# Critical-Infrastructure-Systems-Lab/ldsr

Measured on NVIDIA B200. Metric: EM fits/sec (T~400, restarts x CV folds), higher is better.
Workload: dtype f64

## Files before the change

ldsr_b200/csrc/em_split_kernel.cuh:

```cuda
#pragma once
#include "em_kernel.cuh"

namespace ldsr {

constexpr int SPLIT_NCH = 10;

template <int PQ> __host__ __device__ constexpr int split_nstat() { return 11 + 3 * PQ; }

__host__ __device__ constexpr bool split_w_in_smem(int pq) { return pq <= 4; }
__host__ __device__ inline size_t split_smem_bytes(int pq, int nw, int max_units, int max_uunits) {
    size_t b = 0;
    b += (size_t)max_units * 3 * 32 * 8;
    b += (size_t)2 * nw * 4 * 32 * 8;
    const bool pair = nw % 2 == 0 && nw * (11 + 3 * pq) > 2 * nw * SPLIT_NCH;
    const size_t ch = (size_t)2 * nw * SPLIT_NCH * 32 * 8, st = (size_t)(pair ? nw / 2 : nw) * (11 + 3 * pq) * 32 * 8;
    b += ch > st ? ch : st;
    b += ((size_t)max_units * 4 + 15) & ~size_t(15);
    b += 128;
    b += (size_t)8 * 32 * 8;
    if (split_w_in_smem(pq)) b += (size_t)max_uunits * pq * 32 * 8;
    if (theta_bd_in_smem(pq)) b += (size_t)2 * pq * 32 * 8;
    return b;
}

constexpr int UNIT_M = 1 << 30, UNIT_M1 = 1 << 29, UNIT_US = 1 << 28, UNIT_T0 = UNIT_US - 1;

template <class F> __host__ __device__ inline void split_window_units(int t0, int T, int mseg, int uw, F f) {
    const int end = T < t0 + uw ? T : t0 + uw;
    int t = t0;
    while (t < end) {
        if (t + mseg <= T - 1 && t + mseg <= end) {
            f(t, false);
            t += mseg;
        } else {
            f(t, true);
            t += 1;
        }
    }
}

inline int split_units_upper_bound(const double *y, int T, int mseg, int uw) {
    int n = 0;
    for (int t0 = 0; t0 < T; t0 += uw) {
        bool any = false;
        for (int t = t0; t < T && t < t0 + uw; t++) any = any || (y[t] == y[t]);
        const bool inside = t0 + uw <= T - 1;
        if (!any && inside)
            n += 1;
        else
            split_window_units(t0, T, mseg, uw, [&](int, bool) { n++; });
// ... 82 lines not shown
        const bool obs = (bits >> j) & 1u;
        const double m11 = obs ? k.mc.a11 : k.A2, m12 = obs ? k.mc.a12 : k.Q;
        const double m21 = obs ? k.mc.C2 : 0.0, m22 = obs ? th.R : 1.0;
        nj[j] = n;
        dj[j] = d;
        nn[j] = fma(m11, n, m12 * d);
        dd[j] = fma(m21, n, m22 * d);
        n = nn[j];
        d = dd[j];
    }
    double rho[N], rn[N];
#pragma unroll
    for (int j = 0; j < N; j++) {
        rho[j] = fast_rcp(dd[j]);
        rn[j] = fast_rcp(nn[j]);
    }
#pragma unroll
    for (int j = 0; j < N; j++) {
        const bool obs = (bits >> j) & 1u;
        const double K = obs ? th.C * nj[j] * rho[j] : 0.0;
        const double nu = obs ? th.R * nj[j] : nj[j];
        const double vu = nu * rho[j];
        const double J = k.A * nu * rn[j];
        G.K[j] = K;
        G.rS[j] = obs ? dj[j] * rho[j] : 0.0;
        G.alpha[j] = fma(-k.mc.AC, K, k.A);
        G.J[j] = J;
        G.L[j] = vu * fma(-k.A, J, 1.0);
    }
    G.Vnext = nn[N - 1] * rho[N - 1];
    G.dend = d;
}

template <int PQ, int N>
__device__ __forceinline__ void unit_inputs(const Theta<PQ> &th, unsigned bits, const double *__restrict__ yseg,
                                            const double *__restrict__ useg, const double *__restrict__ vseg,
                                            double (&Bu)[N], double (&ymd)[N], double (&yo)[N],
                                            double (&ur)[N * PQ], double (&vr)[N * PQ]) {
    double yr[N];
    load_vec<N * PQ>(useg, ur);
    load_vec<N * PQ>(vseg, vr);
    load_vec<N>(yseg, yr);
#pragma unroll
    for (int j = 0; j < N; j++) {
        double b = 0.0, dv = 0.0;
#pragma unroll
        for (int i = 0; i < PQ; i++) {
            b = fma(th.b(i), ur[j * PQ + i], b);
            dv = fma(th.d(i), vr[j * PQ + i], dv);
        }
        const bool obs = (bits >> j) & 1u;
        yo[j] = obs ? yr[j] : 0.0;
        Bu[j] = b;
        ymd[j] = yo[j] - dv;
    }
}

struct PieceFwd {
    double Vq, P, q;
    double l0, l1, l2;
    double dprod;
    int shift;
    double PJ, PJ2, G0, GG, Lc;
};

template <int PQ, int UW, int N>
__device__ __forceinline__ void forward_unit_basis(const Theta<PQ> &th, const SplitConst<PQ, UW> &k, unsigned bits,
                                                   const double *__restrict__ yseg, const double *__restrict__ useg,
                                                   const double *__restrict__ vseg, PieceFwd &c) {
    double Bu[N], ymd[N], yo[N];
    {
        double ur[N * PQ], vr[N * PQ];
        unit_inputs<PQ, N>(th, bits, yseg, useg, vseg, Bu, ymd, yo, ur, vr);
    }
    UnitGains<N> G;
    unit_gains<PQ, UW, N>(th, k, bits, c.Vq, G);
    double q[N + 1], P[N + 1];
    q[0] = c.q;
    P[0] = c.P;
#pragma unroll
    for (int j = 0; j < N; j++) {
        const double beta = fma(k.A * G.K[j], ymd[j], Bu[j]);
        q[j + 1] = fma(G.alpha[j], q[j], beta);
        P[j + 1] = G.alpha[j] * P[j];
    }
    double g0[N], gP[N];
#pragma unroll
    for (int j = 0; j < N; j++) {
        const double d0 = fma(-th.C, q[j], ymd[j]);
        const double w0 = G.rS[j] * d0;
        c.l0 = fma(w0, d0, c.l0);
        c.l1 = fma(w0, P[j], c.l1);
        c.l2 = fma(G.rS[j] * P[j], P[j], c.l2);
        const double xu0 = fma(G.K[j], d0, q[j]);
        const double xuP = P[j] * fma(-G.K[j], th.C, 1.0);
        g0[j] = fma(-G.J[j], q[j + 1], xu0);
        gP[j] = fma(-G.J[j], P[j + 1], xuP);
    }
    double pj = c.PJ, pj2 = c.PJ2;
#pragma unroll
    for (int j = 0; j < N; j++) {
        c.G0 = fma(pj, g0[j], c.G0);
        c.GG = fma(pj, gP[j], c.GG);
        c.Lc = fma(pj2, G.L[j], c.Lc);
        pj *= G.J[j];
        pj2 *= G.J[j] * G.J[j];
    }
// ... 52 lines not shown
                lo = fma(k.A, lo, Bu[j]);
                hi = fma(k.A, hi, Bu[4 + j]);
            }
            hh = fma(hh, k.A8, fma(lo, A4, hi));
        }
    }
    if (KEEP_W) {
#pragma unroll
        for (int i = 0; i < PQ; i++) {
            hh = fma(th.b(i), W[i], hh);
            wk[i * 32] = W[i];
        }
    }
    const double AW = k.AW();
    const double qn = fma(AW, c.q, hh);
    const double Pn = AW * c.P;
    const double Vn = fma(k.aVW, c.Vq, k.bVW);
    const double Jc = AW * c.Vq * fast_rcp(Vn);
    const double g0 = fma(-Jc, qn, c.q);
    const double gP = fma(-Jc, Pn, c.P);
    const double L = c.Vq * fma(-AW, Jc, 1.0);
    c.G0 = fma(c.PJ, g0, c.G0);
    c.GG = fma(c.PJ, gP, c.GG);
    c.Lc = fma(c.PJ2, L, c.Lc);
    c.PJ *= Jc;
    c.PJ2 *= Jc * Jc;
    c.q = qn;
    c.P = Pn;
    c.Vq = Vn;
}

template <int PQ, int UW, int N>
__device__ __forceinline__ void smooth_unit(const Theta<PQ> &th, const SplitConst<PQ, UW> &k, unsigned bits, bool last,
                                            const double *__restrict__ yseg, const double *__restrict__ useg,
                                            const double *__restrict__ vseg, double Xq, double Vq, double &Xs1,
                                            double &Vs1, Stats<PQ> &st) {
    constexpr bool KEEP_ROWS = N * PQ <= 16;
    double Bu[N], ymd[N], yo[N];
    double ur[N * PQ], vr[N * PQ];
    unit_inputs<PQ, N>(th, bits, yseg, useg, vseg, Bu, ymd, yo, ur, vr);
    UnitGains<N> G;
    unit_gains<PQ, UW, N>(th, k, bits, Vq, G);
    double xq[N + 1], g[N];
    xq[0] = Xq;
#pragma unroll
    for (int j = 0; j < N; j++) xq[j + 1] = fma(G.alpha[j], xq[j], fma(k.A * G.K[j], ymd[j], Bu[j]));
#pragma unroll
    for (int j = 0; j < N; j++) {
        const double delta = fma(-th.C, xq[j], ymd[j]);
        const double xu = fma(G.K[j], delta, xq[j]);
        g[j] = fma(-G.J[j], xq[j + 1], xu);
    }
    double Xs[N + 1], Vs[N + 1];
    Xs[N] = Xs1;
    Vs[N] = Vs1;
#pragma unroll
    for (int j = N - 1; j >= 0; j--) {
        Xs[j] = fma(G.J[j], Xs[j + 1], g[j]);
        Vs[j] = fma(G.J[j] * G.J[j], Vs[j + 1], G.L[j]);
    }
    if (!KEEP_ROWS) {
        load_vec<N * PQ>(useg, ur);
        load_vec<N * PQ>(vseg, vr);
    }
#pragma unroll
    for (int j = 0; j < N; j++) {
        if (N == 1 && last) {
            st.XT = Xs[j];
            st.VT = Vs[j];
        } else {
            st.Tx1x = fma(Xs[j + 1], Xs[j], st.Tx1x);
            st.Tx1xv = fma(Vs[j + 1], G.J[j], st.Tx1xv);
            st.Txx = fma(Xs[j], Xs[j], st.Txx);
            st.Txxv += Vs[j];
#pragma unroll
            for (int i = 0; i < PQ; i++) {
                st.Tx1u[i] = fma(Xs[j + 1], ur[j * PQ + i], st.Tx1u[i]);
                st.Tux[i] = fma(ur[j * PQ + i], Xs[j], st.Tux[i]);
            }
        }
        const bool obs = (bits >> j) & 1u;
        const double xo = obs ? Xs[j] : 0.0;
        st.Syx = fma(yo[j], xo, st.Syx);
        st.Sxx = fma(xo, xo, st.Sxx);
        st.Sxxv += obs ? Vs[j] : 0.0;
#pragma unroll
        for (int i = 0; i < PQ; i++) st.Sxv[i] = fma(xo, vr[j * PQ + i], st.Sxv[i]);
    }
    Xs1 = Xs[0];
    Vs1 = Vs[0];
}

template <int N> struct ShortConst {
    double AN, aV, bV;
    __device__ __forceinline__ ShortConst(double A, double A2, double Q) {
        double an = 1.0, av = 1.0, sv = 0.0;
#pragma unroll
        for (int j = 0; j < N; j++) {
            an *= A;
            sv = fma(sv, A2, 1.0);
            av *= A2;
        }
        AN = an;
        aV = av;
        bV = Q * sv;
    }
};
template <int PQ, int N>
__device__ __forceinline__ void forward_short_basis(const Theta<PQ> &th, double A, double A2, double Q,
                                                    const double *__restrict__ useg, PieceFwd &c) {
    const ShortConst<N> sc(A, A2, Q);
    double hh = 0.0;
#pragma unroll
    for (int j = 0; j < N; j++) {
        double bu = 0.0;
#pragma unroll
        for (int i = 0; i < PQ; i++) bu = fma(th.b(i), useg[j * PQ + i], bu);
        hh = fma(A, hh, bu);
    }
    const double qn = fma(sc.AN, c.q, hh), Pn = sc.AN * c.P, Vn = fma(sc.aV, c.Vq, sc.bV);
    const double Jc = sc.AN * c.Vq * fast_rcp(Vn);
// ... 125 lines not shown
#pragma unroll
        for (int j = 0; j < 8; j++) Xn[j + 1] = fma(k.A, Xn[j], inp[j]);
        if (!KEEP_U) load_vec<8 * PQ>(blk, uk);
#pragma unroll
        for (int j = 0; j < 8; j++) {
            st.Tx1x = fma(Xn[j + 1], Xn[j], st.Tx1x);
            st.Txx = fma(Xn[j], Xn[j], st.Txx);
#pragma unroll
            for (int i = 0; i < PQ; i++) {
                if (KEEP_W) {
                    tux[i] = fma(uk[j * PQ + i], Xn[j], tux[i]);
                } else {
                    st.Tx1u[i] = fma(Xn[j + 1], uk[j * PQ + i], st.Tx1u[i]);
                    st.Tux[i] = fma(uk[j * PQ + i], Xn[j], st.Tux[i]);
                }
            }
        }
        Xs = Xn[8];
    }
    if (KEEP_W) {
#pragma unroll
        for (int i = 0; i < PQ; i++) {
            double acc = fma(qg0, wk[i * 32], k.A * tux[i]);
#pragma unroll
            for (int j = 0; j < PQ; j++) acc = fma(th.b(j), tuu_w[j * PQ + i], acc);
            st.Tx1u[i] += acc;
            st.Tux[i] += tux[i];
        }
    }
    Xs1 = Xfirst;
    Vs1 = Vfirst;
    cG = G0;
    cH = H0;
}

template <int PQ> __device__ __forceinline__ void stats_store(const Stats<PQ> &st, double *o) {
    o[0 * 32] = st.Syx;
    o[1 * 32] = st.Sxx;
    o[2 * 32] = st.Sxxv;
    o[3 * 32] = st.Tx1x;
    o[4 * 32] = st.Tx1xv;
    o[5 * 32] = st.Txx;
    o[6 * 32] = st.Txxv;
    o[7 * 32] = st.X0;
    o[8 * 32] = st.V0;
    o[9 * 32] = st.XT;
    o[10 * 32] = st.VT;
#pragma unroll
    for (int i = 0; i < PQ; i++) {
        o[(11 + i) * 32] = st.Sxv[i];
        o[(11 + PQ + i) * 32] = st.Tx1u[i];
        o[(11 + 2 * PQ + i) * 32] = st.Tux[i];
    }
}
template <int PQ> __device__ __forceinline__ void stats_add(Stats<PQ> &st, const double *o) {
    st.Syx += o[0 * 32];
    st.Sxx += o[1 * 32];
    st.Sxxv += o[2 * 32];
    st.Tx1x += o[3 * 32];
    st.Tx1xv += o[4 * 32];
    st.Txx += o[5 * 32];
    st.Txxv += o[6 * 32];
    st.X0 += o[7 * 32];
    st.V0 += o[8 * 32];
    st.XT += o[9 * 32];
    st.VT += o[10 * 32];
#pragma unroll
    for (int i = 0; i < PQ; i++) {
        st.Sxv[i] += o[(11 + i) * 32];
        st.Tx1u[i] += o[(11 + PQ + i) * 32];
        st.Tux[i] += o[(11 + 2 * PQ + i) * 32];
    }
}
template <int PQ, int NW> __host__ __device__ constexpr bool split_pairwise() {
    return NW % 2 == 0 && NW * (11 + 3 * PQ) > 2 * NW * SPLIT_NCH;
}
template <int PQ, int NW> __host__ __device__ constexpr int split_st_slots() {
    return split_pairwise<PQ, NW>() ? NW / 2 : NW;
}

struct SplitParams {
    EmParams em;
    int max_units;
    int max_uunits;
    int blob_smem;
    int cost_u, cost_m;
    int *flags;
    int epoch;
    int *ctl;
    const int *order;
    int n_sm;
#ifdef LDSR_PHASE_CLOCKS
    long long *clk;
#endif
};
#ifdef LDSR_PHASE_CLOCKS
#define LDSR_PHASE_MARK(kk)                       \
    do {                                          \
        const long long c_ = clock64();           \
        pc[kk] += c_ - tprev;                     \
        tprev = c_;                               \
    } while (0)
#define LDSR_UNIT_BEGIN() const long long ub_ = clock64()
#define LDSR_UNIT_END(base, u0) pc[(base) + (((u0) & UNIT_M) ? 1 : ((u0) & UNIT_M1) ? 2 : ((u0) & UNIT_US) ? 3 : 0)] += clock64() - ub_
// ... 88 lines not shown
            s_ti = (qi >= 0 && qi < n_tasks) ? SP.order[qi] : -1;
            s_on_sm = r < x ? 2 : 1;
            s_more = 1;
        }
        __syncthreads();
        ti = s_ti;
        if (ti < 0) break;
    } else if (SP.flags) {
        const int W = n_tasks * P.chunk, hi = ((int)blockIdx.x + 1) * slot_len(), w_hi = hi < W ? hi : W;
        if (w_lo >= w_hi) break;
        ti = w_lo / P.chunk;
        const int t_end = (ti + 1) * P.chunk, end = t_end < w_hi ? t_end : w_hi;
        n_it = end - w_lo;
        wait_first = w_lo == ti * P.chunk && end < t_end;
    } else {
        ti = (int)blockIdx.x + seg * (int)gridDim.x;
        if (ti >= n_tasks) break;
    }
    LDSR_CHECK(ti >= 0 && ti < n_tasks && n_it >= 1 && n_it <= P.chunk);
    if (seg > 0) __syncthreads();
    if (wait_first) {
        if (threadIdx.x == 0) flag_wait(SP.flags + ti, SP.epoch);
        __syncthreads();
    }
    const int4 task = P.tasks[ti];
    const SeriesDev S = P.series[task.x];
    const int T = S.T;
    if (threadIdx.x == 0) stage_blob(smem_raw, P.blobs + S.blob_off, (unsigned)S.blob_doubles * 8u, &bar);

    const double *__restrict__ ser = reinterpret_cast<const double *>(smem_raw);
    const double *__restrict__ ys = ser + S.y_off;
    const double *__restrict__ us = ser + S.u_off;
    const double *__restrict__ vs = ser + S.v_off;
    double *const ck = reinterpret_cast<double *>(smem_raw + SP.blob_smem) + lane;
    double *const MC = ck + (size_t)SP.max_units * 96;
    double *const CH = MC + (size_t)NP * 4 * 32;
    double *const ST = CH;
    int *const units =
        reinterpret_cast<int *>(CH - lane + (CH_DOUBLES > ST_DOUBLES ? CH_DOUBLES : ST_DOUBLES));
    int *const pbound = units + ((SP.max_units + 3) & ~3);
    double *const UV = reinterpret_cast<double *>(pbound + 32) + lane;
    double *const WK = UV + 8 * 32;
    double *const TB = WK + (split_w_in_smem(PQ) ? (size_t)SP.max_uunits * PQ * 32 : 0);
    double *const TD = TB + PQ * 32;
    constexpr bool BD_SMEM = theta_bd_in_smem(PQ);

    const bool valid = lane < task.z;
    const int fit = P.active[task.y + (valid ? lane : 0)];
    const int grp = P.f_group[fit];
    const unsigned *__restrict__ mw = P.masks + P.g_mask_off[grp];
    const double *__restrict__ gc = P.gconst + (size_t)grp * gconst_stride(PQ);
    const double *__restrict__ tuu_inv = P.sconst + S.sconst_off;
    const double n_obs = gc[1], inv_n_obs = 1.0 / n_obs;
    constexpr int TL = theta_pad_len<PQ>();
    Theta<PQ> th;
    {
        double g[TL];
#pragma unroll
        for (int i = 0; i < TL; i++) g[i] = ld_l2(P.theta + (size_t)fit * TL + i);
        load_theta<PQ>(th, g);
    }
    th.sb = TB;
    th.sd = TD;
    if (BD_SMEM && warp == 0) {
#pragma unroll
        for (int i = 0; i < PQ; i++) {
            TB[i * 32] = th.B[i];
            TD[i * 32] = th.D[i];
        }
    }
    double l1 = ld_l2(P.l1 + fit), l2 = ld_l2(P.l2 + fit), lik = ld_l2(P.lik + fit);
    int ne = ld_l2(P.ne + fit);
    bool live = valid && (ld_l2(P.done + fit) == 0);
// ... 16 lines not shown
            if (!any && inside) {
                if (lane == 0) units[nu] = t0;
                nu++;
            } else {
                split_window_units(t0, T, MSEG, UW, [&](int t, bool single) {
                    int type = single ? UNIT_M1 : UNIT_M;
#ifndef LDSR_NO_US
                    if (!single && !any_finite(t, MSEG)) type = UNIT_US;
#endif
                    if (lane == 0) units[nu] = t | type;
                    nu++;
                });
            }
        }
        __syncwarp();
        if (lane == 0) {
            int nM = 0;
            for (int i = 0; i < nu; ++i) nM += (units[i] & (UNIT_M | UNIT_M1)) ? 1 : 0;
            int best = nu / 2, best_mis = 1 << 30, mb = 0;
            for (int s = 0; s <= nu; ++s) {
                const int ub = s - mb, ma = nM - mb, uaft = (nu - s) - ma;
                int mis = min(mb + uaft, ub + ma);
                if (s == 0 || s == nu) mis = 1 << 29;
                if (mis < best_mis || (mis == best_mis && abs(2 * s - nu) < abs(2 * best - nu))) {
                    best_mis = mis;
                    best = s;
                }
                if (s < nu && (units[s] & (UNIT_M | UNIT_M1))) mb++;
            }
            split_range<NW>(units, 0, best, SP.cost_u, SP.cost_m, MSEG, pbound);
            split_range<NW>(units, best, nu, SP.cost_u, SP.cost_m, MSEG, pbound + NW);
            LDSR_CHECK(nu <= SP.max_units && (T + UW - 1) / UW <= SP.max_uunits);
            for (int w = 0; w < 2 * NW; ++w) LDSR_CHECK(pbound[w] >= 0 && pbound[w] <= pbound[w + 1] && pbound[w + 1] <= nu);
        }
    }
    mbar_wait(&bar, phase);
    __syncthreads();

#ifdef LDSR_PHASE_CLOCKS
    long long pc[21] = {0, 0, 0, 0, 0, 0, 0, 0, 0, 0, 0, 0, 0, 0, 0, 0, 0, 0, 0, 0, 0}, tprev = clock64();
#endif
    bool counted = false;
    for (int it = 0;; ++it) {
        if (it >= n_it) {
            if (!ranked) break;
            if (!counted) {
                if (threadIdx.x == 0) {
                    atomicAdd(SP.ctl + SHARE_CTL_FINISHED, 1);
                    if (atomicAdd(SP.ctl + SHARE_CTL_DONE + sm_id(2), 1) + 1 < s_on_sm) s_more = 0;
                }
                counted = true;
                __syncthreads();
            }
            if (!s_more) break;
        }
        if (!__any_sync(FULL, live)) break;
        SplitConst<PQ, UW> k;
        k.set(th);

        if (warp == NW - 1) uvar_constants<UW>(k.A2, k.Q, k.aVW, UV);
        LDSR_PHASE_MARK(9);
#pragma unroll 1
        for (int h = 0; h < 2; ++h) {
            const int pj = h * NW + warp;
            if (pj == NP - 1) break;
            double m11 = 1.0, m12 = 0.0, m21 = 0.0, m22 = 1.0;
            const int ua = pbound[pj], ue = pbound[pj + 1];
            for (int un = ua; un < ue; ++un) {
                const int u0 = units[un];
                const int t0 = u0 & UNIT_T0;
                if (u0 & UNIT_M) {
                    compose_var_unit<PQ, UW, MSEG>(th, k, seg_bits(mw, t0, MSEG), m11, m12, m21, m22);
                } else if (u0 & UNIT_M1) {
                    compose_var_unit<PQ, UW, 1>(th, k, seg_bits(mw, t0, 1), m11, m12, m21, m22);
                } else if (u0 & UNIT_US) {
                    const ShortConst<MSEG> sc(k.A, k.A2, k.Q);
                    m11 = fma(sc.aV, m11, sc.bV * m21);
                    m12 = fma(sc.aV, m12, sc.bV * m22);
                } else {
                    m11 = fma(k.aVW, m11, k.bVW * m21);
                    m12 = fma(k.aVW, m12, k.bVW * m22);
                }
            }
            MC[(pj * 4 + 0) * 32] = m11;
            MC[(pj * 4 + 1) * 32] = m12;
            MC[(pj * 4 + 2) * 32] = m21;
            MC[(pj * 4 + 3) * 32] = m22;
        }
        LDSR_PHASE_MARK(0);
        __syncthreads();
        LDSR_PHASE_MARK(1);
        double VinA = th.V1, VinB = th.V1;
        {
            double n = th.V1, d = 1.0;
#pragma unroll
            for (int pj = 0; pj < NP - 1; ++pj) {
                const double m11 = MC[(pj * 4 + 0) * 32], m12 = MC[(pj * 4 + 1) * 32];
                const double m21 = MC[(pj * 4 + 2) * 32], m22 = MC[(pj * 4 + 3) * 32];
                const double nn = fma(m11, n, m12 * d), dd = fma(m21, n, m22 * d);
                n = nn;
                d = dd;
                if (pj + 1 == warp) VinA = n * fast_rcp(d);
                if (pj + 1 == NW + warp) VinB = n * fast_rcp(d);
            }
        }

        LDSR_PHASE_MARK(10);
#pragma unroll 1
        for (int h = 0; h < 2; ++h) {
            const int pj = h * NW + warp;
            const int ua = pbound[pj], ue = pbound[pj + 1];
            PieceFwd c;
            c.Vq = h ? VinB : VinA;
            c.P = 1.0;
            c.q = 0.0;
            c.l0 = c.l1 = c.l2 = 0.0;
            c.dprod = 1.0;
            c.shift = 0;
            c.PJ = c.PJ2 = 1.0;
            c.G0 = c.GG = c.Lc = 0.0;
            bool any_m = false;
            for (int un = ua; un < ue; ++un) {
                const int u0 = units[un];
                const int t0 = u0 & UNIT_T0;
                ck[(un * 3 + 0) * 32] = c.Vq;
                ck[(un * 3 + 1) * 32] = c.q;
                ck[(un * 3 + 2) * 32] = c.P;
                LDSR_UNIT_BEGIN();
                if (u0 & UNIT_M) {
                    any_m = true;
                    forward_unit_basis<PQ, UW, MSEG>(th, k, seg_bits(mw, t0, MSEG), ys + t0, us + t0 * PQ,
                                                     vs + t0 * PQ, c);
                } else if (u0 & UNIT_M1) {
                    any_m = true;
                    forward_unit_basis<PQ, UW, 1>(th, k, seg_bits(mw, t0, 1), ys + t0, us + t0 * PQ, vs + t0 * PQ, c);
                } else if (u0 & UNIT_US) {
                    forward_short_basis<PQ, MSEG>(th, k.A, k.A2, k.Q, us + t0 * PQ, c);
                } else {
                    forward_word_basis<PQ, UW>(th, k, us + t0 * PQ, WK + (size_t)(t0 / UW) * PQ * 32, c);
                }
                LDSR_UNIT_END(13, u0);
            }
            double ld = 0.0;
            if (any_m) ld = fma((double)c.shift, 0.693147180559945309417, log(c.dprod));
            double *o = CH + (size_t)pj * SPLIT_NCH * 32;
            o[0 * 32] = c.P;
            o[1 * 32] = c.q;
            o[2 * 32] = c.l0 + ld;
            o[3 * 32] = c.l1;
            o[4 * 32] = c.l2;
            o[5 * 32] = c.PJ;
            o[6 * 32] = c.G0;
            o[7 * 32] = c.GG;
            o[8 * 32] = c.Lc;
            o[9 * 32] = c.Vq;
        }
        LDSR_PHASE_MARK(2);
        __syncthreads();
        LDSR_PHASE_MARK(3);

        double gk[NP];
        double xinA = 0.0, xinB = 0.0;
        double XrA = 0.0, XrB = 0.0, VrA = 0.0, VrB = 0.0;
        double acc = 0.0;
        double x = th.mu1;
        double vend = th.V1;
        {
#pragma unroll
            for (int pj = 0; pj < NP; ++pj) {
                const double *o = CH + (size_t)pj * SPLIT_NCH * 32;
                if (pj == warp) xinA = x;
                if (pj == NW + warp) xinB = x;
                gk[pj] = fma(o[7 * 32], x, o[6 * 32]);
                const double tC = th.C * x;
                acc += fma(tC, fma(tC, o[4 * 32], -2.0 * o[3 * 32]), o[2 * 32]);
                x = fma(o[0 * 32], x, o[1 * 32]);
                vend = o[9 * 32];
                if (pj == warp) {
                    XrA = x;
                    VrA = vend;
                }
                if (pj == NW + warp) {
                    XrB = x;
                    VrB = vend;
                }
            }
        }
        const double lik_new = (-0.5 * n_obs * LOG_2PI - 0.5 * acc) * inv_n_obs;

        if (live) {
            lik = lik_new;
            ne += 1;
            if (warp == 0 && P.liks) P.liks[(size_t)P.f_user[fit] * P.niter + (ne - 1)] = lik_new;
            const bool conv = (ne >= 3) && (fabs(lik_new - l1) < P.tol) && (fabs(l1 - l2) < P.tol);
            if (conv || ne >= P.niter) live = false;
        }
        if (!__any_sync(FULL, live)) break;

        double Xs1A = 0.0, Vs1A = 0.0, Xs1B = 0.0, Vs1B = 0.0;
        {
            double Xs = x, Vs = vend;
#pragma unroll
            for (int pj = NP - 1; pj >= 0; --pj) {
                if (pj == NW + warp) {
                    Xs1B = Xs;
                    Vs1B = Vs;
                }
                if (pj == warp) {
                    Xs1A = Xs;
                    Vs1A = Vs;
                }
                const double *o = CH + (size_t)pj * SPLIT_NCH * 32;
                const double pjv = o[5 * 32];
                Xs = fma(pjv, Xs, gk[pj]);
                Vs = fma(pjv * pjv, Vs, o[8 * 32]);
            }
        }
        LDSR_PHASE_MARK(4);
        __syncthreads();
        LDSR_PHASE_MARK(5);

        Stats<PQ> st;
        st.zero();
#pragma unroll 1
        for (int h = 1; h >= 0; --h) {
            const int pj = h * NW + warp;
            const int ua = pbound[pj], ue = pbound[pj + 1];
            const double xin = h ? xinB : xinA;
            double Xs1 = h ? Xs1B : Xs1A, Vs1 = h ? Vs1B : Vs1A;
            double Xr = h ? XrB : XrA, Vr = h ? VrB : VrA;
            double cG = 0.0, cH = 0.0;
            bool in_run = false;
            for (int un = ue - 1; un >= ua; --un) {
                const int u0 = units[un];
                const int t0 = u0 & UNIT_T0;
                const double Vq = ck[(un * 3 + 0) * 32];
                const double Xq = fma(ck[(un * 3 + 2) * 32], xin, ck[(un * 3 + 1) * 32]);
                LDSR_UNIT_BEGIN();
                if (u0 & UNIT_M) {
                    smooth_unit<PQ, UW, MSEG>(th, k, seg_bits(mw, t0, MSEG), false, ys + t0, us + t0 * PQ,
                                              vs + t0 * PQ, Xq, Vq, Xs1, Vs1, st);
                    in_run = false;
                } else if (u0 & UNIT_M1) {
                    smooth_unit<PQ, UW, 1>(th, k, seg_bits(mw, t0, 1), t0 == T - 1, ys + t0, us + t0 * PQ,
                                           vs + t0 * PQ, Xq, Vq, Xs1, Vs1, st);
                    in_run = false;
                } else {
                    if (!in_run) {
                        const double rv = fast_rcp(Vr);
                        cG = (Xs1 - Xr) * rv;
                        cH = (Vs1 - Vr) * rv * rv;
                        in_run = true;
                    }
                    if (u0 & UNIT_US)
                        smooth_short<PQ, MSEG>(th, k.A, k.A2, k.Q, us + t0 * PQ, Xq, Vq, cG, cH, Xs1, Vs1, st);
                    else
                    smooth_word<PQ, UW>(th, k, us + t0 * PQ, UV, WK + (size_t)(t0 / UW) * PQ * 32,
                                        P.uwin + S.uwin_off + (size_t)(t0 / UW) * PQ * PQ, Xq, Vq, cG, cH, Xs1, Vs1, st);
                }
                LDSR_UNIT_END(17, u0);
                Xr = Xq;
                Vr = Vq;
            }
            if (ua == 0 && ue > 0) {
                st.X0 = Xs1;
                st.V0 = Vs1;
            }
        }
        LDSR_PHASE_MARK(6);
        if (ranked && it + 1 >= n_it && threadIdx.x == 0)
            s_more = ld_relaxed(SP.ctl + SHARE_CTL_FINISHED) + (counted ? 0 : 1) < n_tasks;
        if (!PAIR) {
            stats_store<PQ>(st, ST + (size_t)warp * NST * 32);
            __syncthreads();
            LDSR_PHASE_MARK(7);
            st.zero();
#pragma unroll
            for (int w = 0; w < NW; ++w) stats_add<PQ>(st, ST + (size_t)w * NST * 32);
        } else {
            if (warp >= NW / 2) stats_store<PQ>(st, ST + (size_t)(warp - NW / 2) * NST * 32);
            __syncthreads();
            if (warp < NW / 2) {
                stats_add<PQ>(st, ST + (size_t)warp * NST * 32);
                stats_store<PQ>(st, ST + (size_t)warp * NST * 32);
            }
            __syncthreads();
            if (warp == 0) {
                st.zero();
#pragma unroll
                for (int w = 0; w < NW / 2; ++w) stats_add<PQ>(st, ST + (size_t)w * NST * 32);
            }
        }
        LDSR_PHASE_MARK(11);
        if (!PAIR) {
            if (live) mstep_from_stats<PQ, true>(st, gc, tuu_inv, T, th);
        } else {
            double g[TL];
            if (warp == 0) {
                if (BD_SMEM) {
#pragma unroll
                    for (int i = 0; i < PQ; i++) {
                        th.B[i] = TB[i * 32];
                        th.D[i] = TD[i * 32];
                    }
                }
                if (live) mstep_from_stats<PQ, true>(st, gc, tuu_inv, T, th);
                if (BD_SMEM) {
#pragma unroll
                    for (int i = 0; i < PQ; i++) {
                        TB[i * 32] = th.B[i];
                        TD[i * 32] = th.D[i];
                    }
                }
                store_theta<PQ>(th, g);
#pragma unroll
                for (int i = 0; i < TL; i++) ST[i * 32] = g[i];
            }
            __syncthreads();
            if (warp != 0) {
#pragma unroll
                for (int i = 0; i < TL; i++) g[i] = ST[i * 32];
                load_theta<PQ>(th, g);
            }
        }
        if (live) {
            l2 = l1;
            l1 = lik;
        }
        LDSR_PHASE_MARK(8);
    }
#ifdef LDSR_PHASE_CLOCKS
    if (lane == 0 && SP.clk)
        for (int i = 0; i < 21; i++) SP.clk[((size_t)blockIdx.x * NW + warp) * 21 + i] = pc[i];
#endif

    if (ranked && !counted && threadIdx.x == 0) {
        atomicAdd(SP.ctl + SHARE_CTL_FINISHED, 1);
        atomicAdd(SP.ctl + SHARE_CTL_DONE + sm_id(2), 1);
    }
    if (BD_SMEM && warp == 0) {
#pragma unroll
        for (int i = 0; i < PQ; i++) {
            th.B[i] = TB[i * 32];
            th.D[i] = TD[i * 32];
        }
    }
    if (warp == 0 && valid) {
        store_theta<PQ>(th, P.theta + (size_t)fit * TL);
        P.l1[fit] = l1;
        P.l2[fit] = l2;
        P.lik[fit] = lik;
        P.ne[fit] = ne;
        P.done[fit] = live ? 0 : 1;
    }
    if (SP.flags) {
        if (w_lo % P.chunk != 0 && warp == 0) {
            __threadfence();
            __syncwarp();
            if (lane == 0) flag_raise(SP.flags + w_lo / P.chunk, SP.epoch);
        }
        w_lo += n_it;
    }
// ... 5 lines not shown
```

ldsr_b200/csrc/ldsr_abi.cu:

```cuda
#include "../../include/ldsr_b200.h"
#include "generic_kernels.cuh"
#include "kernel_table.h"
#include "r_rng.cuh"
#include "scan_kernels.cuh"

#include <algorithm>
#include <atomic>
#include <chrono>
#include <condition_variable>
#include <cmath>
#include <cstdarg>
#include <cstdio>
#include <cstdlib>
#include <cstring>
#include <functional>
#include <memory>
#include <mutex>
#include <numeric>
#include <string>
#include <thread>
#include <vector>

namespace ldsr {

// ... 801 lines not shown
            sp.cost_u = P->kt->split_uw * 22;
            sp.cost_m = P->kt->split_mseg * 168;
#ifdef LDSR_PHASE_CLOCKS
            if (!sp_clk_last) cudaMalloc(&sp_clk_last, sizeof(long long) * 4096 * 21 * 8);
            sp.clk = (c == 1 && grid <= 4096) ? sp_clk_last : nullptr;
#endif
            sp.flags = share_slots > 0 ? P->d_share_flags : nullptr;
            sp.epoch = ++P->share_epoch;
            sp.ctl = share_ranked ? P->d_share_ctl : nullptr;
            sp.order = P->d_share_order;
            sp.n_sm = P->n_sm;
            cudaError_t le = (grid <= 2 * P->n_sm || sp.flags) ? P->kt->em_split_wide(sp, grid, smem, st)
                                                               : P->kt->em_split(sp, grid, smem, st);
            if (le == cudaErrorCooperativeLaunchTooLarge && sp.flags) {
                cudaGetLastError();
                share_slots = 0;
                share_ranked = false;
                sp.flags = nullptr;
                sp.ctl = nullptr;
                grid = plain_grid;
                le = grid <= 2 * P->n_sm ? P->kt->em_split_wide(sp, grid, smem, st) : P->kt->em_split(sp, grid, smem, st);
            }
            CU(le);
        } else {
            CU(P->kt->em_chunk(ep, grid, smem, st));
        }
        if (stats) CU(cudaEventRecord(evs.back(), st));
#ifdef LDSR_PHASE_CLOCKS
        if (use_split && c == 1 && grid <= 4096) {
            const int nw = P->kt->split_nw;
            std::vector<long long> h((size_t)grid * nw * 21);
            cudaStreamSynchronize(st);
            cudaMemcpy(h.data(), sp_clk_last, h.size() * sizeof(long long), cudaMemcpyDeviceToHost);
            static const char *names[21] = {"P1 loops", "B1 wait", "P2", "B2 wait", "chain+stop", "B2' wait",
                                            "P4", "B3 wait", "M-step", "constants", "prefix", "reduce",
                                            "-", "P2 U words", "P2 M units", "P2 M1 units",
                                            "P2 US units", "P4 U words", "P4 M units", "P4 M1 units", "P4 US units"};
            std::fprintf(stderr, "[ldsr] phase clocks of launch 1 (cycles per iteration, mean over %d CTAs), per warp:\n", grid);
            for (int i = 0; i < 21; i++) {
                std::fprintf(stderr, "[ldsr]   %-14s", names[i]);
                for (int w = 0; w < nw; w++) {
                    double sum = 0;
                    for (int b = 0; b < grid; b++) sum += (double)h[((size_t)b * nw + w) * 21 + i];
                    std::fprintf(stderr, " %9.0f", sum / grid / chunk);
                }
                std::fprintf(stderr, "\n");
            }
        }
#endif
        launches++;
        enq++;
    }
    if (!sync_each) {
        CU(cudaMemcpyAsync(P->h_counts, P->d_counts, (size_t)2 * max_chunks * sizeof(int), cudaMemcpyDeviceToHost, st));
        CU(cudaStreamSynchronize(st));
        if (abort_flag && abort_flag->load()) return fail(LDSR_ERR_INTERRUPTED, "interrupted");
    } else {
        CU(cudaStreamSynchronize(st));
    }
    static const bool trace_chunks = std::getenv("LDSR_TIMING") != nullptr;
    for (int c = 0; c < enq; ++c) {
        if (P->h_counts[2 * c + 1] > 0) chunks++;
        if (stats) {
            float ms = 0.f;
            CU(cudaEventElapsedTime(&ms, evs[2 * c], evs[2 * c + 1]));
            if (P->h_counts[2 * c + 1] > 0) em_ms += ms;
            if (trace_chunks)
                std::fprintf(stderr, "[ldsr] chunk %d: %d tasks, %d live fits, %.3f ms\n", c, P->h_counts[2 * c],
                             P->h_counts[2 * c + 1], ms);
// ... 1462 lines not shown
```

Baseline: 735,600.

## Compute chain once in one warp, split M-step across two warps

Previously every warp redundantly ran the forward and backward chain over all pieces. Now only the last warp runs them and publishes per-piece prefix results to shared memory, and the other warps read their slots after a barrier. In the non-pair path, the M-step is divided so warp 0 does the observation block and warp 1 the transition block, each publishing its theta half to shared memory, which every warp then reloads after an extra barrier. The variance-prefix loop also exits early once a warp's own piece is reached. This removes redundant serial work and shortens the serial M-step, at the cost of an additional __syncthreads and shared-memory round trips.

```diff
diff --git a/ldsr_b200/csrc/em_split_kernel.cuh b/ldsr_b200/csrc/em_split_kernel.cuh
--- a/ldsr_b200/csrc/em_split_kernel.cuh
+++ b/ldsr_b200/csrc/em_split_kernel.cuh
@@ -590,10 +590,14 @@
         o[(11 + 2 * PQ + i) * 32] = st.Tux[i];
     }
 }
-template <int PQ> __device__ __forceinline__ void stats_add(Stats<PQ> &st, const double *o) {
+template <int PQ> __device__ __forceinline__ void stats_add_obs(Stats<PQ> &st, const double *o) {
     st.Syx += o[0 * 32];
     st.Sxx += o[1 * 32];
     st.Sxxv += o[2 * 32];
+#pragma unroll
+    for (int i = 0; i < PQ; i++) st.Sxv[i] += o[(11 + i) * 32];
+}
+template <int PQ> __device__ __forceinline__ void stats_add_trans(Stats<PQ> &st, const double *o) {
     st.Tx1x += o[3 * 32];
     st.Tx1xv += o[4 * 32];
     st.Txx += o[5 * 32];
@@ -604,9 +608,39 @@
     st.VT += o[10 * 32];
 #pragma unroll
     for (int i = 0; i < PQ; i++) {
-        st.Sxv[i] += o[(11 + i) * 32];
         st.Tx1u[i] += o[(11 + PQ + i) * 32];
         st.Tux[i] += o[(11 + 2 * PQ + i) * 32];
+    }
+}
+template <int PQ> __device__ __forceinline__ void stats_add(Stats<PQ> &st, const double *o) {
+    stats_add_obs<PQ>(st, o);
+    stats_add_trans<PQ>(st, o);
+}
+template <int PQ> __device__ __forceinline__ void theta_publish_obs(const Theta<PQ> &th, double *o) {
+    o[0 * 32] = th.C;
+    o[1 * 32] = th.R;
+#pragma unroll
+    for (int i = 0; i < PQ; i++) o[(11 + i) * 32] = th.D[i];
+}
+template <int PQ> __device__ __forceinline__ void theta_publish_trans(const Theta<PQ> &th, double *o) {
+    o[3 * 32] = th.A;
+    o[4 * 32] = th.Q;
+    o[5 * 32] = th.mu1;
+    o[6 * 32] = th.V1;
+#pragma unroll
+    for (int i = 0; i < PQ; i++) o[(11 + PQ + i) * 32] = th.B[i];
+}
+template <int PQ> __device__ __forceinline__ void theta_load_published(Theta<PQ> &th, const double *o) {
+    th.C = o[0 * 32];
+    th.R = o[1 * 32];
+    th.A = o[3 * 32];
+    th.Q = o[4 * 32];
+    th.mu1 = o[5 * 32];
+    th.V1 = o[6 * 32];
+#pragma unroll
+    for (int i = 0; i < PQ; i++) {
+        th.D[i] = o[(11 + i) * 32];
+        th.B[i] = o[(11 + PQ + i) * 32];
     }
 }
 template <int PQ, int NW> __host__ __device__ constexpr bool split_pairwise() {
@@ -913,6 +947,7 @@
             double n = th.V1, d = 1.0;
 #pragma unroll
             for (int pj = 0; pj < NP - 1; ++pj) {
+                if (pj == NW + warp) break;
                 const double m11 = MC[(pj * 4 + 0) * 32], m12 = MC[(pj * 4 + 1) * 32];
                 const double m21 = MC[(pj * 4 + 2) * 32], m22 = MC[(pj * 4 + 3) * 32];
                 const double nn = fma(m11, n, m12 * d), dd = fma(m21, n, m22 * d);
@@ -977,34 +1012,39 @@
         __syncthreads();
         LDSR_PHASE_MARK(3);
 
-        double gk[NP];
-        double xinA = 0.0, xinB = 0.0;
-        double XrA = 0.0, XrB = 0.0, VrA = 0.0, VrB = 0.0;
-        double acc = 0.0;
-        double x = th.mu1;
-        double vend = th.V1;
-        {
+        double *const CX = MC;
+        constexpr int CX_XS1 = NP + 1, CX_VS1 = 2 * NP + 1, CX_LIK = 3 * NP + 1;
+        static_assert(CX_LIK < NP * 4, "chain results fit the variance-map slots");
+        if (warp == NW - 1) {
+            double gk[NP];
+            double acc = 0.0;
+            double x = th.mu1;
 #pragma unroll
             for (int pj = 0; pj < NP; ++pj) {
                 const double *o = CH + (size_t)pj * SPLIT_NCH * 32;
-                if (pj == warp) xinA = x;
-                if (pj == NW + warp) xinB = x;
+                CX[pj * 32] = x;
                 gk[pj] = fma(o[7 * 32], x, o[6 * 32]);
                 const double tC = th.C * x;
                 acc += fma(tC, fma(tC, o[4 * 32], -2.0 * o[3 * 32]), o[2 * 32]);
                 x = fma(o[0 * 32], x, o[1 * 32]);
-                vend = o[9 * 32];
-                if (pj == warp) {
-                    XrA = x;
-                    VrA = vend;
-                }
-                if (pj == NW + warp) {
-                    XrB = x;
-                    VrB = vend;
-                }
-            }
-        }
-        const double lik_new = (-0.5 * n_obs * LOG_2PI - 0.5 * acc) * inv_n_obs;
+            }
+            CX[NP * 32] = x;
+            CX[CX_LIK * 32] = (-0.5 * n_obs * LOG_2PI - 0.5 * acc) * inv_n_obs;
+            double Xs = x, Vs = CH[((NP - 1) * SPLIT_NCH + 9) * 32];
+#pragma unroll
+            for (int pj = NP - 1; pj >= 0; --pj) {
+                CX[(CX_XS1 + pj) * 32] = Xs;
+                CX[(CX_VS1 + pj) * 32] = Vs;
+                const double *o = CH + (size_t)pj * SPLIT_NCH * 32;
+                const double pjv = o[5 * 32];
+                Xs = fma(pjv, Xs, gk[pj]);
+                Vs = fma(pjv * pjv, Vs, o[8 * 32]);
+            }
+        }
+        const double VrA = CH[(warp * SPLIT_NCH + 9) * 32], VrB = CH[((NW + warp) * SPLIT_NCH + 9) * 32];
+        LDSR_PHASE_MARK(4);
+        __syncthreads();
+        const double lik_new = CX[CX_LIK * 32];
 
         if (live) {
             lik = lik_new;
@@ -1014,28 +1054,10 @@
             if (conv || ne >= P.niter) live = false;
         }
         if (!__any_sync(FULL, live)) break;
-
-        double Xs1A = 0.0, Vs1A = 0.0, Xs1B = 0.0, Vs1B = 0.0;
-        {
-            double Xs = x, Vs = vend;
-#pragma unroll
-            for (int pj = NP - 1; pj >= 0; --pj) {
-                if (pj == NW + warp) {
-                    Xs1B = Xs;
-                    Vs1B = Vs;
-                }
-                if (pj == warp) {
-                    Xs1A = Xs;
-                    Vs1A = Vs;
-                }
-                const double *o = CH + (size_t)pj * SPLIT_NCH * 32;
-                const double pjv = o[5 * 32];
-                Xs = fma(pjv, Xs, gk[pj]);
-                Vs = fma(pjv * pjv, Vs, o[8 * 32]);
-            }
-        }
-        LDSR_PHASE_MARK(4);
-        __syncthreads();
+        const double xinA = CX[warp * 32], xinB = CX[(NW + warp) * 32];
+        const double XrA = CX[(warp + 1) * 32], XrB = CX[(NW + warp + 1) * 32];
+        const double Xs1A = CX[(CX_XS1 + warp) * 32], Xs1B = CX[(CX_XS1 + NW + warp) * 32];
+        const double Vs1A = CX[(CX_VS1 + warp) * 32], Vs1B = CX[(CX_VS1 + NW + warp) * 32];
         LDSR_PHASE_MARK(5);
 
         Stats<PQ> st;
@@ -1092,9 +1114,25 @@
             stats_store<PQ>(st, ST + (size_t)warp * NST * 32);
             __syncthreads();
             LDSR_PHASE_MARK(7);
+            static_assert(NW >= 2, "one warp per block of the M-step");
             st.zero();
-#pragma unroll
-            for (int w = 0; w < NW; ++w) stats_add<PQ>(st, ST + (size_t)w * NST * 32);
+            if (warp == 0) {
+#pragma unroll
+                for (int w = 0; w < NW; ++w) stats_add_obs<PQ>(st, ST + (size_t)w * NST * 32);
+                LDSR_PHASE_MARK(11);
+                if (live) mstep_obs_block<PQ, true>(st, gc, th);
+                theta_publish_obs<PQ>(th, ST);
+            } else if (warp == 1) {
+#pragma unroll
+                for (int w = 0; w < NW; ++w) stats_add_trans<PQ>(st, ST + (size_t)w * NST * 32);
+                LDSR_PHASE_MARK(11);
+                if (live) mstep_trans_block<PQ, true>(st, tuu_inv, T, th);
+                theta_publish_trans<PQ>(th, ST);
+            }
+            LDSR_PHASE_MARK(8);
+            __syncthreads();
+            theta_load_published<PQ>(th, ST);
+            LDSR_PHASE_MARK(12);
         } else {
             if (warp >= NW / 2) stats_store<PQ>(st, ST + (size_t)(warp - NW / 2) * NST * 32);
             __syncthreads();
@@ -1108,11 +1146,7 @@
 #pragma unroll
                 for (int w = 0; w < NW / 2; ++w) stats_add<PQ>(st, ST + (size_t)w * NST * 32);
             }
-        }
-        LDSR_PHASE_MARK(11);
-        if (!PAIR) {
-            if (live) mstep_from_stats<PQ, true>(st, gc, tuu_inv, T, th);
-        } else {
+            LDSR_PHASE_MARK(11);
             double g[TL];
             if (warp == 0) {
                 if (BD_SMEM) {
@@ -1140,12 +1174,12 @@
                 for (int i = 0; i < TL; i++) g[i] = ST[i * 32];
                 load_theta<PQ>(th, g);
             }
+            LDSR_PHASE_MARK(8);
         }
         if (live) {
             l2 = l1;
             l1 = lik;
         }
-        LDSR_PHASE_MARK(8);
     }
 #ifdef LDSR_PHASE_CLOCKS
     if (lane == 0 && SP.clk)
diff --git a/ldsr_b200/csrc/ldsr_abi.cu b/ldsr_b200/csrc/ldsr_abi.cu
--- a/ldsr_b200/csrc/ldsr_abi.cu
+++ b/ldsr_b200/csrc/ldsr_abi.cu
@@ -857,9 +857,9 @@
             std::vector<long long> h((size_t)grid * nw * 21);
             cudaStreamSynchronize(st);
             cudaMemcpy(h.data(), sp_clk_last, h.size() * sizeof(long long), cudaMemcpyDeviceToHost);
-            static const char *names[21] = {"P1 loops", "B1 wait", "P2", "B2 wait", "chain+stop", "B2' wait",
+            static const char *names[21] = {"P1 loops", "B1 wait", "P2", "B2 wait", "chain", "B2' wait+stop",
                                             "P4", "B3 wait", "M-step", "constants", "prefix", "reduce",
-                                            "-", "P2 U words", "P2 M units", "P2 M1 units",
+                                            "B4 wait+theta", "P2 U words", "P2 M units", "P2 M1 units",
                                             "P2 US units", "P4 U words", "P4 M units", "P4 M1 units", "P4 US units"};
             std::fprintf(stderr, "[ldsr] phase clocks of launch 1 (cycles per iteration, mean over %d CTAs), per warp:\n", grid);
             for (int i = 0; i < 21; i++) {
```

After: 769,000 (median of 6 runs). +4.5%, better.

## Group units into same-type runs and prefetch next unit's rows in forward/smooth

Applied to the files above, without the earlier changes.

Precomputes runs of consecutive same-type units per piece so the compose, forward and smooth loops dispatch once per run instead of once per unit. Within each run, the y/u/v rows, mask bits and checkpoint values for the next unit are loaded while the current unit computes (for PQ<=4), hiding global-load latency. This costs extra shared memory for the run table, extra registers for the prefetched rows, and a limit of fewer than 2^15 units.

```diff
diff --git a/ldsr_b200/csrc/em_split_kernel.cuh b/ldsr_b200/csrc/em_split_kernel.cuh
--- a/ldsr_b200/csrc/em_split_kernel.cuh
+++ b/ldsr_b200/csrc/em_split_kernel.cuh
@@ -16,6 +16,7 @@
     const size_t ch = (size_t)2 * nw * SPLIT_NCH * 32 * 8, st = (size_t)(pair ? nw / 2 : nw) * (11 + 3 * pq) * 32 * 8;
     b += ch > st ? ch : st;
     b += ((size_t)max_units * 4 + 15) & ~size_t(15);
+    b += ((size_t)max_units * 8 + 15) & ~size_t(15);
     b += 128;
     b += (size_t)8 * 32 * 8;
     if (split_w_in_smem(pq)) b += (size_t)max_uunits * pq * 32 * 8;
@@ -164,25 +165,32 @@
     G.dend = d;
 }
 
+struct SeriesRows {
+    const double *__restrict__ y, *__restrict__ u, *__restrict__ v;
+};
+__host__ __device__ constexpr bool split_prefetch(int pq) { return pq <= 4; }
+template <int PQ, int N> struct UnitRows {
+    double y[N], u[N * PQ], v[N * PQ];
+    __device__ __forceinline__ void load(const SeriesRows &s, int t) {
+        load_vec<N * PQ>(s.u + t * PQ, u);
+        load_vec<N * PQ>(s.v + t * PQ, v);
+        load_vec<N>(s.y + t, y);
+    }
+};
+
 template <int PQ, int N>
-__device__ __forceinline__ void unit_inputs(const Theta<PQ> &th, unsigned bits, const double *__restrict__ yseg,
-                                            const double *__restrict__ useg, const double *__restrict__ vseg,
-                                            double (&Bu)[N], double (&ymd)[N], double (&yo)[N],
-                                            double (&ur)[N * PQ], double (&vr)[N * PQ]) {
-    double yr[N];
-    load_vec<N * PQ>(useg, ur);
-    load_vec<N * PQ>(vseg, vr);
-    load_vec<N>(yseg, yr);
+__device__ __forceinline__ void unit_inputs(const Theta<PQ> &th, unsigned bits, const UnitRows<PQ, N> &R,
+                                            double (&Bu)[N], double (&ymd)[N], double (&yo)[N]) {
 #pragma unroll
     for (int j = 0; j < N; j++) {
         double b = 0.0, dv = 0.0;
 #pragma unroll
         for (int i = 0; i < PQ; i++) {
-            b = fma(th.b(i), ur[j * PQ + i], b);
-            dv = fma(th.d(i), vr[j * PQ + i], dv);
+            b = fma(th.b(i), R.u[j * PQ + i], b);
+            dv = fma(th.d(i), R.v[j * PQ + i], dv);
         }
         const bool obs = (bits >> j) & 1u;
-        yo[j] = obs ? yr[j] : 0.0;
+        yo[j] = obs ? R.y[j] : 0.0;
         Bu[j] = b;
         ymd[j] = yo[j] - dv;
     }
@@ -195,16 +203,18 @@
     int shift;
     double PJ, PJ2, G0, GG, Lc;
 };
+__device__ __forceinline__ void store_checkpoint(double *__restrict__ ck, int un, const PieceFwd &c) {
+    ck[(un * 3 + 0) * 32] = c.Vq;
+    ck[(un * 3 + 1) * 32] = c.q;
+    ck[(un * 3 + 2) * 32] = c.P;
+}
 
 template <int PQ, int UW, int N>
 __device__ __forceinline__ void forward_unit_basis(const Theta<PQ> &th, const SplitConst<PQ, UW> &k, unsigned bits,
-                                                   const double *__restrict__ yseg, const double *__restrict__ useg,
-                                                   const double *__restrict__ vseg, PieceFwd &c) {
+                                                   UnitRows<PQ, N> &R, const SeriesRows &src, int tn, PieceFwd &c) {
     double Bu[N], ymd[N], yo[N];
-    {
-        double ur[N * PQ], vr[N * PQ];
-        unit_inputs<PQ, N>(th, bits, yseg, useg, vseg, Bu, ymd, yo, ur, vr);
-    }
+    unit_inputs<PQ, N>(th, bits, R, Bu, ymd, yo);
+    if (split_prefetch(PQ)) R.load(src, tn);
     UnitGains<N> G;
     unit_gains<PQ, UW, N>(th, k, bits, c.Vq, G);
     double q[N + 1], P[N + 1];
@@ -323,13 +333,13 @@
 
 template <int PQ, int UW, int N>
 __device__ __forceinline__ void smooth_unit(const Theta<PQ> &th, const SplitConst<PQ, UW> &k, unsigned bits, bool last,
-                                            const double *__restrict__ yseg, const double *__restrict__ useg,
-                                            const double *__restrict__ vseg, double Xq, double Vq, double &Xs1,
-                                            double &Vs1, Stats<PQ> &st) {
+                                            UnitRows<PQ, N> &R, const SeriesRows &src, int t, int tn, double Xq,
+                                            double Vq, double &Xs1, double &Vs1, Stats<PQ> &st) {
     constexpr bool KEEP_ROWS = N * PQ <= 16;
     double Bu[N], ymd[N], yo[N];
-    double ur[N * PQ], vr[N * PQ];
-    unit_inputs<PQ, N>(th, bits, yseg, useg, vseg, Bu, ymd, yo, ur, vr);
+    double(&ur)[N * PQ] = R.u;
+    double(&vr)[N * PQ] = R.v;
+    unit_inputs<PQ, N>(th, bits, R, Bu, ymd, yo);
     UnitGains<N> G;
     unit_gains<PQ, UW, N>(th, k, bits, Vq, G);
     double xq[N + 1], g[N];
@@ -351,8 +361,8 @@
         Vs[j] = fma(G.J[j] * G.J[j], Vs[j + 1], G.L[j]);
     }
     if (!KEEP_ROWS) {
-        load_vec<N * PQ>(useg, ur);
-        load_vec<N * PQ>(vseg, vr);
+        load_vec<N * PQ>(src.u + t * PQ, ur);
+        load_vec<N * PQ>(src.v + t * PQ, vr);
     }
 #pragma unroll
     for (int j = 0; j < N; j++) {
@@ -378,6 +388,7 @@
 #pragma unroll
         for (int i = 0; i < PQ; i++) st.Sxv[i] = fma(xo, vr[j * PQ + i], st.Sxv[i]);
     }
+    if (split_prefetch(PQ)) R.load(src, tn);
     Xs1 = Xs[0];
     Vs1 = Vs[0];
 }
@@ -569,6 +580,91 @@
     Vs1 = Vfirst;
     cG = G0;
     cH = H0;
+}
+
+
+template <int PQ, int UW, int N>
+__device__ __forceinline__ void compose_var_run(const Theta<PQ> &th, const SplitConst<PQ, UW> &k,
+                                                const unsigned *__restrict__ mw, int t, int n, double &m11,
+                                                double &m12, double &m21, double &m22) {
+    unsigned bits = seg_bits(mw, t, N);
+#pragma unroll 1
+    for (int i = 1; i <= n; ++i) {
+        const int tn = i < n ? t + N : t;
+        const unsigned bn = seg_bits(mw, tn, N);
+        compose_var_unit<PQ, UW, N>(th, k, bits, m11, m12, m21, m22);
+        t = tn;
+        bits = bn;
+    }
+}
+
+template <int PQ, int UW, int N>
+__device__ __forceinline__ void forward_run(const Theta<PQ> &th, const SplitConst<PQ, UW> &k,
+                                            const unsigned *__restrict__ mw, const SeriesRows &src, int t, int un,
+                                            int n, double *__restrict__ ck, PieceFwd &c) {
+    constexpr bool PF = split_prefetch(PQ);
+    UnitRows<PQ, N> R;
+    unsigned bits = 0;
+    if (PF) {
+        R.load(src, t);
+        bits = seg_bits(mw, t, N);
+    }
+#pragma unroll 1
+    for (const int ue = un + n; un < ue; ++un) {
+        store_checkpoint(ck, un, c);
+        const int tn = un + 1 < ue ? t + N : t;
+        if (!PF) {
+            R.load(src, t);
+            bits = seg_bits(mw, t, N);
+        }
+        const unsigned bn = PF ? seg_bits(mw, tn, N) : 0u;
+        forward_unit_basis<PQ, UW, N>(th, k, bits, R, src, tn, c);
+        t = tn;
+        bits = bn;
+    }
+}
+
+template <int PQ, int UW, int N>
+__device__ __forceinline__ void smooth_run(const Theta<PQ> &th, const SplitConst<PQ, UW> &k,
+                                           const unsigned *__restrict__ mw, const SeriesRows &src, int T, int t,
+                                           int un, int n, const double *__restrict__ ck, double xin, double &Xs1,
+                                           double &Vs1, double &Xr, double &Vr, Stats<PQ> &st) {
+    constexpr bool PF = split_prefetch(PQ);
+    int u = un + n - 1;
+    t += (n - 1) * N;
+    UnitRows<PQ, N> R;
+    unsigned bits = 0;
+    double Vq = 0.0, q = 0.0, P = 0.0;
+    const auto fetch = [&](int v, int tv, unsigned &b, double &V, double &qv, double &Pv) {
+        b = seg_bits(mw, tv, N);
+        V = ck[(v * 3 + 0) * 32];
+        qv = ck[(v * 3 + 1) * 32];
+        Pv = ck[(v * 3 + 2) * 32];
+    };
+    if (PF) {
+        R.load(src, t);
+        fetch(u, t, bits, Vq, q, P);
+    }
+#pragma unroll 1
+    for (; u >= un; --u) {
+        const int tn = u > un ? t - N : t;
+        if (!PF) {
+            R.load(src, t);
+            fetch(u, t, bits, Vq, q, P);
+        }
+        unsigned bn = 0;
+        double Vqn = 0.0, qn = 0.0, Pn = 0.0;
+        if (PF) fetch(u > un ? u - 1 : u, tn, bn, Vqn, qn, Pn);
+        const double Xq = fma(P, xin, q);
+        smooth_unit<PQ, UW, N>(th, k, bits, t == T - 1, R, src, t, tn, Xq, Vq, Xs1, Vs1, st);
+        Xr = Xq;
+        Vr = Vq;
+        t = tn;
+        bits = bn;
+        Vq = Vqn;
+        q = qn;
+        P = Pn;
+    }
 }
 
 template <int PQ> __device__ __forceinline__ void stats_store(const Stats<PQ> &st, double *o) {
@@ -761,13 +857,17 @@
     const double *__restrict__ ys = ser + S.y_off;
     const double *__restrict__ us = ser + S.u_off;
     const double *__restrict__ vs = ser + S.v_off;
+    const SeriesRows src{ys, us, vs};
     double *const ck = reinterpret_cast<double *>(smem_raw + SP.blob_smem) + lane;
     double *const MC = ck + (size_t)SP.max_units * 96;
     double *const CH = MC + (size_t)NP * 4 * 32;
     double *const ST = CH;
     int *const units =
         reinterpret_cast<int *>(CH - lane + (CH_DOUBLES > ST_DOUBLES ? CH_DOUBLES : ST_DOUBLES));
-    int *const pbound = units + ((SP.max_units + 3) & ~3);
+    int *const runs = units + ((SP.max_units + 3) & ~3);
+    int *const pbound = runs + ((2 * SP.max_units + 3) & ~3);
+    int *const rbound = pbound + 16;
+    static_assert(NP + 1 <= 16, "piece bounds and run bounds share 32 ints");
     double *const UV = reinterpret_cast<double *>(pbound + 32) + lane;
     double *const WK = UV + 8 * 32;
     double *const TB = WK + (split_w_in_smem(PQ) ? (size_t)SP.max_uunits * PQ * 32 : 0);
@@ -850,6 +950,21 @@
             split_range<NW>(units, best, nu, SP.cost_u, SP.cost_m, MSEG, pbound + NW);
             LDSR_CHECK(nu <= SP.max_units && (T + UW - 1) / UW <= SP.max_uunits);
             for (int w = 0; w < 2 * NW; ++w) LDSR_CHECK(pbound[w] >= 0 && pbound[w] <= pbound[w + 1] && pbound[w + 1] <= nu);
+            LDSR_CHECK(nu < (1 << 15));
+            int nr = 0;
+            for (int pj = 0; pj < NP; ++pj) {
+                rbound[pj] = nr;
+#pragma unroll 1
+                for (int a = pbound[pj], e; a < pbound[pj + 1]; a = e) {
+                    const int type = units[a] & ~UNIT_T0;
+                    for (e = a + 1; e < pbound[pj + 1] && (units[e] & ~UNIT_T0) == type; ++e) {
+                    }
+                    runs[2 * nr] = units[a];
+                    runs[2 * nr + 1] = a | (e - a) << 16;
+                    nr++;
+                }
+            }
+            rbound[NP] = nr;
         }
     }
     mbar_wait(&bar, phase);
@@ -883,21 +998,27 @@
             const int pj = h * NW + warp;
             if (pj == NP - 1) break;
             double m11 = 1.0, m12 = 0.0, m21 = 0.0, m22 = 1.0;
-            const int ua = pbound[pj], ue = pbound[pj + 1];
-            for (int un = ua; un < ue; ++un) {
-                const int u0 = units[un];
+#pragma unroll 1
+            for (int r = rbound[pj]; r < rbound[pj + 1]; ++r) {
+                const int u0 = runs[2 * r], n = runs[2 * r + 1] >> 16;
                 const int t0 = u0 & UNIT_T0;
                 if (u0 & UNIT_M) {
-                    compose_var_unit<PQ, UW, MSEG>(th, k, seg_bits(mw, t0, MSEG), m11, m12, m21, m22);
+                    compose_var_run<PQ, UW, MSEG>(th, k, mw, t0, n, m11, m12, m21, m22);
                 } else if (u0 & UNIT_M1) {
-                    compose_var_unit<PQ, UW, 1>(th, k, seg_bits(mw, t0, 1), m11, m12, m21, m22);
+                    compose_var_run<PQ, UW, 1>(th, k, mw, t0, n, m11, m12, m21, m22);
                 } else if (u0 & UNIT_US) {
                     const ShortConst<MSEG> sc(k.A, k.A2, k.Q);
-                    m11 = fma(sc.aV, m11, sc.bV * m21);
-                    m12 = fma(sc.aV, m12, sc.bV * m22);
+#pragma unroll 1
+                    for (int i = 0; i < n; ++i) {
+                        m11 = fma(sc.aV, m11, sc.bV * m21);
+                        m12 = fma(sc.aV, m12, sc.bV * m22);
+                    }
                 } else {
-                    m11 = fma(k.aVW, m11, k.bVW * m21);
-                    m12 = fma(k.aVW, m12, k.bVW * m22);
+#pragma unroll 1
+                    for (int i = 0; i < n; ++i) {
+                        m11 = fma(k.aVW, m11, k.bVW * m21);
+                        m12 = fma(k.aVW, m12, k.bVW * m22);
+                    }
                 }
             }
             MC[(pj * 4 + 0) * 32] = m11;
@@ -927,7 +1048,6 @@
 #pragma unroll 1
         for (int h = 0; h < 2; ++h) {
             const int pj = h * NW + warp;
-            const int ua = pbound[pj], ue = pbound[pj + 1];
             PieceFwd c;
             c.Vq = h ? VinB : VinA;
             c.P = 1.0;
@@ -938,24 +1058,30 @@
             c.PJ = c.PJ2 = 1.0;
             c.G0 = c.GG = c.Lc = 0.0;
             bool any_m = false;
-            for (int un = ua; un < ue; ++un) {
-                const int u0 = units[un];
+#pragma unroll 1
+            for (int r = rbound[pj]; r < rbound[pj + 1]; ++r) {
+                const int u0 = runs[2 * r], ua = runs[2 * r + 1] & 0xffff, n = runs[2 * r + 1] >> 16;
                 const int t0 = u0 & UNIT_T0;
-                ck[(un * 3 + 0) * 32] = c.Vq;
-                ck[(un * 3 + 1) * 32] = c.q;
-                ck[(un * 3 + 2) * 32] = c.P;
                 LDSR_UNIT_BEGIN();
                 if (u0 & UNIT_M) {
                     any_m = true;
-                    forward_unit_basis<PQ, UW, MSEG>(th, k, seg_bits(mw, t0, MSEG), ys + t0, us + t0 * PQ,
-                                                     vs + t0 * PQ, c);
+                    forward_run<PQ, UW, MSEG>(th, k, mw, src, t0, ua, n, ck, c);
                 } else if (u0 & UNIT_M1) {
                     any_m = true;
-                    forward_unit_basis<PQ, UW, 1>(th, k, seg_bits(mw, t0, 1), ys + t0, us + t0 * PQ, vs + t0 * PQ, c);
+                    forward_run<PQ, UW, 1>(th, k, mw, src, t0, ua, n, ck, c);
                 } else if (u0 & UNIT_US) {
-                    forward_short_basis<PQ, MSEG>(th, k.A, k.A2, k.Q, us + t0 * PQ, c);
+#pragma unroll 1
+                    for (int i = 0; i < n; ++i) {
+                        store_checkpoint(ck, ua + i, c);
+                        forward_short_basis<PQ, MSEG>(th, k.A, k.A2, k.Q, us + (t0 + i * MSEG) * PQ, c);
+                    }
                 } else {
-                    forward_word_basis<PQ, UW>(th, k, us + t0 * PQ, WK + (size_t)(t0 / UW) * PQ * 32, c);
+#pragma unroll 1
+                    for (int i = 0; i < n; ++i) {
+                        const int t = t0 + i * UW;
+                        store_checkpoint(ck, ua + i, c);
+                        forward_word_basis<PQ, UW>(th, k, us + t * PQ, WK + (size_t)(t / UW) * PQ * 32, c);
+                    }
                 }
                 LDSR_UNIT_END(13, u0);
             }
@@ -1049,19 +1175,16 @@
             double Xr = h ? XrB : XrA, Vr = h ? VrB : VrA;
             double cG = 0.0, cH = 0.0;
             bool in_run = false;
-            for (int un = ue - 1; un >= ua; --un) {
-                const int u0 = units[un];
+#pragma unroll 1
+            for (int r = rbound[pj + 1] - 1; r >= rbound[pj]; --r) {
+                const int u0 = runs[2 * r], ur = runs[2 * r + 1] & 0xffff, n = runs[2 * r + 1] >> 16;
                 const int t0 = u0 & UNIT_T0;
-                const double Vq = ck[(un * 3 + 0) * 32];
-                const double Xq = fma(ck[(un * 3 + 2) * 32], xin, ck[(un * 3 + 1) * 32]);
                 LDSR_UNIT_BEGIN();
                 if (u0 & UNIT_M) {
-                    smooth_unit<PQ, UW, MSEG>(th, k, seg_bits(mw, t0, MSEG), false, ys + t0, us + t0 * PQ,
-                                              vs + t0 * PQ, Xq, Vq, Xs1, Vs1, st);
+                    smooth_run<PQ, UW, MSEG>(th, k, mw, src, T, t0, ur, n, ck, xin, Xs1, Vs1, Xr, Vr, st);
                     in_run = false;
                 } else if (u0 & UNIT_M1) {
-                    smooth_unit<PQ, UW, 1>(th, k, seg_bits(mw, t0, 1), t0 == T - 1, ys + t0, us + t0 * PQ,
-                                           vs + t0 * PQ, Xq, Vq, Xs1, Vs1, st);
+                    smooth_run<PQ, UW, 1>(th, k, mw, src, T, t0, ur, n, ck, xin, Xs1, Vs1, Xr, Vr, st);
                     in_run = false;
                 } else {
                     if (!in_run) {
@@ -1070,15 +1193,31 @@
                         cH = (Vs1 - Vr) * rv * rv;
                         in_run = true;
                     }
-                    if (u0 & UNIT_US)
-                        smooth_short<PQ, MSEG>(th, k.A, k.A2, k.Q, us + t0 * PQ, Xq, Vq, cG, cH, Xs1, Vs1, st);
-                    else
-                    smooth_word<PQ, UW>(th, k, us + t0 * PQ, UV, WK + (size_t)(t0 / UW) * PQ * 32,
-                                        P.uwin + S.uwin_off + (size_t)(t0 / UW) * PQ * PQ, Xq, Vq, cG, cH, Xs1, Vs1, st);
+                    if (u0 & UNIT_US) {
+#pragma unroll 1
+                        for (int un = ur + n - 1; un >= ur; --un) {
+                            const int t = t0 + (un - ur) * MSEG;
+                            const double Vq = ck[(un * 3 + 0) * 32];
+                            const double Xq = fma(ck[(un * 3 + 2) * 32], xin, ck[(un * 3 + 1) * 32]);
+                            smooth_short<PQ, MSEG>(th, k.A, k.A2, k.Q, us + t * PQ, Xq, Vq, cG, cH, Xs1, Vs1, st);
+                            Xr = Xq;
+                            Vr = Vq;
+                        }
+                    } else {
+#pragma unroll 1
+                        for (int un = ur + n - 1; un >= ur; --un) {
+                            const int t = t0 + (un - ur) * UW;
+                            const double Vq = ck[(un * 3 + 0) * 32];
+                            const double Xq = fma(ck[(un * 3 + 2) * 32], xin, ck[(un * 3 + 1) * 32]);
+                            smooth_word<PQ, UW>(th, k, us + t * PQ, UV, WK + (size_t)(t / UW) * PQ * 32,
+                                                P.uwin + S.uwin_off + (size_t)(t / UW) * PQ * PQ, Xq, Vq, cG, cH, Xs1,
+                                                Vs1, st);
+                            Xr = Xq;
+                            Vr = Vq;
+                        }
+                    }
                 }
                 LDSR_UNIT_END(17, u0);
-                Xr = Xq;
-                Vr = Vq;
             }
             if (ua == 0 && ue > 0) {
                 st.X0 = Xs1;
```

New measurement: 734,600 before, 739,200 after (median of 6 runs). About the same (+0.6%).
